# yezhen17/3DIoUMatch

Hardware: AMD Instinct MI355X
Metric: scenes/sec train-step (ScanNet 40k pts, 256 proposals) (higher is better)
Workload: dtype f32

## Files before the change

3dioumatch_amd/_lib.py:

```python
import ctypes
import os

_HERE = os.path.dirname(os.path.abspath(__file__))
LIB_PATH = os.path.join(_HERE, "lib3dioumatch_hip%s.so" % os.environ.get("PN2_LIB_SUFFIX", ""))

_c_int, _c_float, _vp, _sz = ctypes.c_int, ctypes.c_float, ctypes.c_void_p, ctypes.c_size_t


class MlpOperand(ctypes.Structure):
    _fields_ = [("mode", _c_int), ("x", _vp), ("dz", _vp), ("scale", _vp), ("shift", _vp), ("mean", _vp),
                ("invstd", _vp), ("coef", _vp), ("argmax", _vp), ("ns", _c_int), ("groups", _c_int),
                ("lin_w", _vp)]


_op = ctypes.POINTER(MlpOperand)

_SIGNATURES = {
    "pn2_furthest_point_sampling": [_c_int, _c_int, _c_int, _vp, _vp, _vp, _vp],
    "pn2_furthest_point_sampling_ws": [_c_int, _c_int, _c_int, _vp, _vp, _vp, _sz, _vp],
    "pn2_fps_workspace_bytes": [_c_int, _c_int, _c_int],
    "pn2_gather_points": [_c_int, _c_int, _c_int, _c_int, _vp, _vp, _vp, _vp],
    "pn2_gather_points_grad": [_c_int, _c_int, _c_int, _c_int, _vp, _vp, _vp, _vp],
    "pn2_ball_query": [_c_int, _c_int, _c_int, _c_float, _c_int, _vp, _vp, _vp, _vp, _sz, _vp],
    "pn2_ball_query_workspace_bytes": [_c_int, _c_int, _c_int, _c_int],
    "pn2_group_points": [_c_int, _c_int, _c_int, _c_int, _c_int, _vp, _vp, _vp, _vp],
    "pn2_group_points_grad": [_c_int, _c_int, _c_int, _c_int, _c_int, _vp, _vp, _vp, _vp],
    "pn2_three_nn": [_c_int, _c_int, _c_int, _vp, _vp, _vp, _vp, _vp],
    "pn2_three_interpolate": [_c_int, _c_int, _c_int, _c_int, _vp, _vp, _vp, _vp, _vp],
    "pn2_three_interpolate_affine_supported": [_c_int, _c_int, _c_int],
    "pn2_three_interpolate_affine": [_c_int, _c_int, _c_int, _c_int, _vp, _vp, _vp, _vp, _vp, _vp, _vp],
    "pn2_three_interpolate_affine_ld": [_c_int, _c_int, _c_int, _c_int, _vp, _vp, _vp, _vp, _c_int, _vp, _vp,
                                        _vp],
    "pn2_three_interpolate_rows_into": [_c_int, _c_int, _c_int, _c_int, _vp, _vp, _vp, _vp, _c_int, _c_int,
                                        _vp, _c_int, _c_int, _vp],
    "pn2_three_interpolate_grad": [_c_int, _c_int, _c_int, _c_int, _vp, _vp, _vp, _vp, _vp],
    "pn2_three_nn_weights": [ctypes.c_longlong, _vp, _vp, _vp],
    "pn2_multi_copy": [_c_int, _vp, ctypes.c_longlong, _vp],
    "pn2_group_inverse_supported": [_c_int, _c_int, _c_int],
    "pn2_group_inverse_entries": [_c_int, _c_int],
    "pn2_group_inverse_build": [_c_int, _c_int, _c_int, _c_int, _vp, _vp, _vp],
    "pn2_group_points_grad_sorted": [_c_int, _c_int, _c_int, _c_int, _c_int, _vp, _c_int, _c_int, _vp,
                                     _vp, _vp],
    "pn2_three_interpolate_into": [_c_int, _c_int, _c_int, _c_int, _vp, _vp, _vp, _vp, _c_int, _vp],
    "pn2_three_interpolate_grad_from": [_c_int, _c_int, _c_int, _c_int, _vp, _c_int, _vp, _vp, _vp, _vp],
    "pn2_query_and_group": [_c_int, _c_int, _c_int, _c_int, _c_float, _c_int, _c_int, _vp, _vp,
                            _vp, _vp, _vp, _vp, _sz, _vp],
    "pn2_group_concat": [_c_int, _c_int, _c_int, _c_int, _c_float, _c_int, _c_int, _vp, _vp,
                         _vp, _vp, _vp, _vp],
    "pn2_grid_bytes": [_c_int, _c_int],
    "pn2_grid_launch_order": [_c_int, _c_int, _vp, _vp, _vp, _vp],
    "pn2_grid_build": [_c_int, _c_int, _c_float, _vp, _vp, _sz, _vp],
    "pn2_ball_query_prebuilt": [_c_int, _c_int, _c_int, _c_float, _c_int, _vp, _vp, _vp, _vp, _sz, _vp],
    "pn2_query_and_group_prebuilt": [_c_int, _c_int, _c_int, _c_int, _c_float, _c_int, _c_int, _vp,
                                     _vp, _vp, _vp, _vp, _vp, _sz, _vp],
    "pn2_query_and_group_picks": [_c_int, _c_int, _c_int, _c_int, _c_float, _c_int, _c_int, _vp,
                                  _vp, _vp, _vp, _vp, _vp, _sz, _vp],
    "pn2_fps_grid_supported": [_c_int],
    "pn2_furthest_point_sampling_grid": [_c_int, _c_int, _c_int, _vp, _vp, _vp, _sz, _c_float, _vp,
                                         _sz, _vp],
    "pn2_fps_ties_supported": [_c_int],
    "pn2_furthest_point_sampling_ties": [_c_int, _c_int, _c_int, _vp, _vp, _vp, _sz, _c_float, _vp,
                                         _sz, _vp, _vp],
    "pn2_furthest_point_sampling_prefix": [_c_int, _c_int, _c_int, _vp, _vp, _vp, _sz, _vp, _vp],
    "pn2_error_string": [_c_int],
    "mlp_bn_workspace_floats": [_c_int, _c_int, _c_int],
    "mlp_bn_train_stats": [_c_int, _c_int, _c_int, _vp, _vp, _vp, _c_float, _c_float, _vp, _vp, _vp,
                           _vp, _vp, _vp, _vp, _vp, _vp],
    "mlp_bn_eval_coeff": [_c_int, _vp, _vp, _c_float, _vp, _vp, _vp, _vp, _vp, _vp, _vp],
    "mlp_bn_relu_apply": [_c_int, _c_int, _c_int, _vp, _vp, _vp, _vp, _vp],
    "mlp_bn_relu_pool": [_c_int, _c_int, _c_int, _c_int, _vp, _vp, _vp, _vp, _vp, _vp, _vp],
    "mlp_bn_relu_backward": [_c_int, _c_int, _c_int, _c_int, _vp, _vp, _vp, _vp, _vp, _vp, _vp, _vp,
                             _vp, _vp, _vp, _vp, _vp, _vp],
    "mlp_bn_relu_pool_backward": [_c_int, _c_int, _c_int, _c_int, _c_int, _vp, _vp, _vp, _vp, _vp,
                                  _vp, _vp, _vp, _vp, _vp, _vp, _vp, _vp, _vp, _vp, _vp],
    "mlp_bn_relu_backward_stats": [_c_int, _c_int, _c_int, _c_int, _vp, _vp, _vp, _vp, _vp, _vp,
                                   _vp, _vp, _vp, _vp, _vp, _vp, _vp],
    "mlp_gemm_forward": [_c_int] * 4 + [_vp, _vp, _op, _vp, _vp, _vp],
    "mlp_gemm_forward_small": [_c_int] * 4 + [_vp, _c_int, _vp, _op, _vp, _vp, _vp],
    "mlp_gemm_forward_stats_parts": [_c_int, _c_int, _c_int, _c_int, _vp],
    "mlp_bn_finalize_pairs": [_c_int, _c_int, _c_int, _vp, _vp, _vp, _c_float, _c_float, _vp, _vp,
                              _vp, _vp, _vp, _vp, _vp, _vp],
# ... 149 lines not shown
```

3dioumatch_amd/csrc/pn2_interp.hip:

```cpp
#include "common.h"

namespace {

constexpr int kNNTile = 1024;

__global__ void __launch_bounds__(256)
three_nn_kernel(int n, int m, const float *__restrict__ unknown,
                const float *__restrict__ known, float *__restrict__ dist2,
                int *__restrict__ idx) {
  __shared__ float4 tile[kNNTile];
  const BlockId blk = xcd_block_id();
  const int b = blk.y;
  const int j = blk.x * 256 + threadIdx.x;
  const bool live = j < n;
  const float *kn = known + (size_t)b * m * 3;
  float ux = 0.f, uy = 0.f, uz = 0.f;
  if (live) {
    const float *u = unknown + ((size_t)b * n + j) * 3;
    ux = u[0]; uy = u[1]; uz = u[2];
  }
  float best1 = __builtin_inff(), best2 = __builtin_inff(), best3 = __builtin_inff();
  int besti1 = 0, besti2 = 0, besti3 = 0;
  for (int base = 0; base < m; base += kNNTile) {
    const int cnt = m - base < kNNTile ? m - base : kNNTile;
// ... 145 lines not shown
                                 __fmul_rn(src[ii[t][1]], ww[t][1])),
                       __fmul_rn(src[ii[t][2]], ww[t][2]));
    float *dst = out + (size_t)b * out_bstride + (size_t)l * n + j0;
    if (JP == 4) {
      *reinterpret_cast<float4 *>(dst) = make_float4(r[0], r[1], r[2], r[3]);
    } else {
      dst[0] = r[0];
    }
  }
}

template <int CPW>
__global__ void __launch_bounds__(256)
three_interpolate_lds_kernel(int c, int m, int n, const float *__restrict__ points,
                             const int *__restrict__ idx, const float *__restrict__ weight,
                             float *__restrict__ out, size_t out_bstride, RowCopy rc) {
  extern __shared__ __attribute__((aligned(16))) float rows[];
  const BlockId blk = xcd_block_id();
  const int ygroups = (c + CPW - 1) / CPW;
  if (blk.y >= ygroups) {
    copy_rows<4>(rc, n, blk.z, blk.y - ygroups, (int)gridDim.y - ygroups, blk.x);
    return;
  }
  const int b = blk.z, l0 = blk.y * CPW;
  const int nc = c - l0 < CPW ? c - l0 : CPW;
  const float *src = points + ((size_t)b * c + l0) * m;
  for (int t = threadIdx.x; t < nc * m; t += 256) rows[t] = src[t];
  __syncthreads();
  const int j0 = (blk.x * 256 + threadIdx.x) * 4;
  if (j0 >= n) return;
  const int4 *ib = reinterpret_cast<const int4 *>(idx + ((size_t)b * n + j0) * 3);
  const float4 *wb = reinterpret_cast<const float4 *>(weight + ((size_t)b * n + j0) * 3);
  const int4 i0 = ib[0], i1 = ib[1], i2 = ib[2];
  const float4 w0 = wb[0], w1 = wb[1], w2 = wb[2];
  const int ii[12] = {i0.x, i0.y, i0.z, i0.w, i1.x, i1.y, i1.z, i1.w, i2.x, i2.y, i2.z, i2.w};
  const float ww[12] = {w0.x, w0.y, w0.z, w0.w, w1.x, w1.y, w1.z, w1.w, w2.x, w2.y, w2.z, w2.w};
#pragma unroll
  for (int cc = 0; cc < CPW; ++cc) {
    if (cc < nc) {
      const float *row = rows + cc * m;
      float r[4];
#pragma unroll
      for (int t = 0; t < 4; ++t)
        r[t] = __fadd_rn(__fadd_rn(__fmul_rn(row[ii[3 * t]], ww[3 * t]),
                                   __fmul_rn(row[ii[3 * t + 1]], ww[3 * t + 1])),
                         __fmul_rn(row[ii[3 * t + 2]], ww[3 * t + 2]));
      typedef float ti_f4 __attribute__((ext_vector_type(4)));
      __builtin_nontemporal_store(ti_f4{r[0], r[1], r[2], r[3]},
                                  reinterpret_cast<ti_f4 *>(out + (size_t)b * out_bstride + (size_t)(l0 + cc) * n + j0));
    }
  }
}

template <int CPW>
__global__ void __launch_bounds__(256)
three_interpolate_affine_lds_kernel(int c, int m, int n, const float *__restrict__ points,
                                    const int *__restrict__ idx, const float *__restrict__ weight,
                                    const float *__restrict__ aw, int aw_ld,
                                    const float *__restrict__ ax, float *__restrict__ out) {
  extern __shared__ __attribute__((aligned(16))) float rows[];
  const BlockId blk = xcd_block_id();
  const int b = blk.z, l0 = blk.y * CPW;
  const int nc = c - l0 < CPW ? c - l0 : CPW;
  const float *src = points + ((size_t)b * c + l0) * m;
  for (int t = threadIdx.x; t < nc * m; t += 256) rows[t] = src[t];
  __syncthreads();
  const int j0 = (blk.x * 256 + threadIdx.x) * 4;
  if (j0 >= n) return;
  const int4 *ib = reinterpret_cast<const int4 *>(idx + ((size_t)b * n + j0) * 3);
  const float4 *wb = reinterpret_cast<const float4 *>(weight + ((size_t)b * n + j0) * 3);
  const int4 i0 = ib[0], i1 = ib[1], i2 = ib[2];
  const float4 w0 = wb[0], w1 = wb[1], w2 = wb[2];
  const int ii[12] = {i0.x, i0.y, i0.z, i0.w, i1.x, i1.y, i1.z, i1.w, i2.x, i2.y, i2.z, i2.w};
  const float ww[12] = {w0.x, w0.y, w0.z, w0.w, w1.x, w1.y, w1.z, w1.w, w2.x, w2.y, w2.z, w2.w};
  const float *axb = ax + (size_t)b * 3 * n + j0;
  const float4 x0 = *reinterpret_cast<const float4 *>(axb), x1 = *reinterpret_cast<const float4 *>(axb + n),
               x2 = *reinterpret_cast<const float4 *>(axb + 2 * (size_t)n);
  const float xs[4][3] = {{x0.x, x1.x, x2.x}, {x0.y, x1.y, x2.y}, {x0.z, x1.z, x2.z}, {x0.w, x1.w, x2.w}};
#pragma unroll
  for (int cc = 0; cc < CPW; ++cc) {
    if (cc < nc) {
      const float *row = rows + cc * m;
      const float *awr = aw + (size_t)(l0 + cc) * aw_ld;
      const float a0 = awr[0], a1 = awr[1], a2 = awr[2];
      float r[4];
#pragma unroll
      for (int t = 0; t < 4; ++t) {
        const float interp = __fadd_rn(__fadd_rn(__fmul_rn(row[ii[3 * t]], ww[3 * t]),
                                                 __fmul_rn(row[ii[3 * t + 1]], ww[3 * t + 1])),
                                       __fmul_rn(row[ii[3 * t + 2]], ww[3 * t + 2]));
        const float affine = __fadd_rn(__fadd_rn(__fmul_rn(a0, xs[t][0]), __fmul_rn(a1, xs[t][1])),
                                       __fmul_rn(a2, xs[t][2]));
        r[t] = __fadd_rn(affine, interp);
      }
      typedef float ti_f4 __attribute__((ext_vector_type(4)));
      __builtin_nontemporal_store(ti_f4{r[0], r[1], r[2], r[3]},
                                  reinterpret_cast<ti_f4 *>(out + ((size_t)b * c + l0 + cc) * n + j0));
    }
  }
}

template <int CPW>
__global__ void __launch_bounds__(256)
three_interpolate_grad_lds_kernel(int c, int n, int m, const float *__restrict__ grad_out,
                                  size_t g_bstride, const int *__restrict__ idx,
                                  const float *__restrict__ weight,
                                  float *__restrict__ grad_points) {
  extern __shared__ __attribute__((aligned(16))) float lds[];
  const BlockId blk = xcd_block_id();
  const int b = blk.y, l0 = blk.x * CPW;
  const int nc = c - l0 < CPW ? c - l0 : CPW;
  for (int t = threadIdx.x; t < 4 * CPW * m; t += 256) lds[t] = 0.f;
  __syncthreads();
  float *rows = lds + (threadIdx.x >> 6) * CPW * m;
  for (int j = threadIdx.x; j < n; j += 256) {
    const int *ib = idx + ((size_t)b * n + j) * 3;
    const float *wb = weight + ((size_t)b * n + j) * 3;
    const int i1 = ib[0], i2 = ib[1], i3 = ib[2];
    const float w1 = wb[0], w2 = wb[1], w3 = wb[2];
#pragma unroll
    for (int cc = 0; cc < CPW; ++cc) {
      if (cc < nc) {
        const float g = grad_out[(size_t)b * g_bstride + (size_t)(l0 + cc) * n + j];
        float *row = rows + cc * m;
        atomicAdd(row + i1, __fmul_rn(g, w1));
        atomicAdd(row + i2, __fmul_rn(g, w2));
        atomicAdd(row + i3, __fmul_rn(g, w3));
      }
    }
  }
  __syncthreads();
  float *dst = grad_points + ((size_t)b * c + l0) * m;
  const int span = CPW * m;
  for (int t = threadIdx.x; t < nc * m; t += 256)
    dst[t] = __fadd_rn(__fadd_rn(__fadd_rn(lds[t], lds[span + t]), lds[2 * span + t]), lds[3 * span + t]);
}

__global__ void __launch_bounds__(256)
three_interpolate_grad_kernel(int c, int n, int m, const float *__restrict__ grad_out,
                              size_t g_bstride, const int *__restrict__ idx,
                              const float *__restrict__ weight, float *__restrict__ grad_points) {
  const BlockId blk = xcd_block_id();
  const int b = blk.z;
  const int j = blk.x * 256 + threadIdx.x;
  if (j >= n) return;
  const int *ib = idx + ((size_t)b * n + j) * 3;
  const float *wb = weight + ((size_t)b * n + j) * 3;
  const int i1 = ib[0], i2 = ib[1], i3 = ib[2];
  const float w1 = wb[0], w2 = wb[1], w3 = wb[2];
  for (int l = blk.y; l < c; l += gridDim.y) {
    const float g = grad_out[(size_t)b * g_bstride + (size_t)l * n + j];
// ... 41 lines not shown
    dim3 grid(pn2_ceil_div(n, 1024), pn2_ceil_div(c, CPW) + copy_groups, b);
    hipLaunchKernelGGL(three_interpolate_lds_kernel<CPW>, grid, dim3(256),
                       sizeof(float) * (size_t)CPW * m, stream, c, m, n, points, idx, weight, out,
                       out_bstride, rc);
    return pn2_launch_status();
  }
  const int ygroups = interp_channel_groups(c);
  if (vec) {
    dim3 grid(pn2_ceil_div(n, 1024), ygroups + copy_groups, b);
    hipLaunchKernelGGL(three_interpolate_kernel<4>, grid, dim3(256), 0, stream, c, m, n, points,
                       idx, weight, out, out_bstride, ygroups, rc);
  } else {
    dim3 grid(pn2_ceil_div(n, 256), ygroups + copy_groups, b);
    hipLaunchKernelGGL(three_interpolate_kernel<1>, grid, dim3(256), 0, stream, c, m, n, points,
                       idx, weight, out, out_bstride, ygroups, rc);
  }
  return pn2_launch_status();
}

static int interpolate_grad_run(int b, int c, int n, int m, const float *grad_out, size_t g_bstride,
                                const int *idx, const float *weight, float *grad_points,
                                hipStream_t stream) {
  if (b <= 0 || c <= 0 || m <= 0) return 0;
  if (n > 0 && m <= 1024) {
    constexpr int CPW = 4;
    hipLaunchKernelGGL(three_interpolate_grad_lds_kernel<CPW>, dim3(pn2_ceil_div(c, CPW), b),
                       dim3(256), sizeof(float) * 4 * (size_t)CPW * m, stream, c, n, m, grad_out,
                       g_bstride, idx, weight, grad_points);
    return pn2_launch_status();
  }
  const int e = pn2_zero_async(grad_points, sizeof(float) * (size_t)b * c * m, stream);
  if (e != 0) return e;
  if (n <= 0) return 0;
  dim3 grid(pn2_ceil_div(n, 256), interp_channel_groups(c), b);
  hipLaunchKernelGGL(three_interpolate_grad_kernel, grid, dim3(256), 0, stream, c, n, m, grad_out,
                     g_bstride, idx, weight, grad_points);
  return pn2_launch_status();
}

PN2_API int pn2_three_interpolate_affine_supported(int c, int m, int n) {
  return c > 0 && m > 0 && m <= 2048 && n >= 4 && n % 4 == 0;
}

PN2_API int pn2_three_interpolate_affine_ld(int b, int c, int m, int n, const float *points, const int *idx,
                                            const float *weight, const float *affine_w, int affine_w_ld,
                                            const float *affine_x, float *out, void *stream_) {
  if (b <= 0) return 0;
  if (!pn2_three_interpolate_affine_supported(c, m, n) || !affine_w || !affine_x || affine_w_ld < 3 ||
      (reinterpret_cast<size_t>(out) & 15) || (reinterpret_cast<size_t>(affine_x) & 15) ||
      (reinterpret_cast<size_t>(idx) & 15) || (reinterpret_cast<size_t>(weight) & 15))
    return (int)hipErrorInvalidValue;
  constexpr int CPW = 8;
  dim3 grid(pn2_ceil_div(n, 1024), pn2_ceil_div(c, CPW), b);
  hipLaunchKernelGGL(three_interpolate_affine_lds_kernel<CPW>, grid, dim3(256),
                     sizeof(float) * (size_t)CPW * m, (hipStream_t)stream_, c, m, n, points, idx, weight,
                     affine_w, affine_w_ld, affine_x, out);
  return pn2_launch_status();
}

PN2_API int pn2_three_interpolate_affine(int b, int c, int m, int n, const float *points, const int *idx,
                                         const float *weight, const float *affine_w,
                                         const float *affine_x, float *out, void *stream_) {
  return pn2_three_interpolate_affine_ld(b, c, m, n, points, idx, weight, affine_w, 3, affine_x, out,
                                         stream_);
}

PN2_API int pn2_three_interpolate(int b, int c, int m, int n, const float *points,
                                  const int *idx, const float *weight, float *out,
                                  void *stream_) {
  return interpolate_run(b, c, m, n, points, idx, weight, out, (size_t)c * n, (hipStream_t)stream_);
}

PN2_API int pn2_three_interpolate_grad(int b, int c, int n, int m, const float *grad_out,
                                       const int *idx, const float *weight, float *grad_points,
                                       void *stream_) {
  return interpolate_grad_run(b, c, n, m, grad_out, (size_t)c * n, idx, weight, grad_points,
                              (hipStream_t)stream_);
}

PN2_API int pn2_three_interpolate_into(int b, int c, int m, int n, const float *points,
                                       const int *idx, const float *weight, float *out,
                                       int c_total, void *stream_) {
  if (c_total < c) return (int)hipErrorInvalidValue;
  return interpolate_run(b, c, m, n, points, idx, weight, out, (size_t)c_total * n,
                         (hipStream_t)stream_);
}

PN2_API int pn2_three_interpolate_rows_into(int b, int c, int m, int n, const float *points,
                                            const int *idx, const float *weight, float *out,
                                            int c_total, int channel0, const float *rows, int rows_c,
                                            int rows_channel0, void *stream_) {
  if (b <= 0 || n <= 0) return 0;
  if (c <= 0 || rows_c <= 0 || !rows || channel0 < 0 || rows_channel0 < 0 ||
      channel0 + c > c_total || rows_channel0 + rows_c > c_total ||
      (channel0 < rows_channel0 + rows_c && rows_channel0 < channel0 + c))
    return (int)hipErrorInvalidValue;
  const size_t bstride = (size_t)c_total * n;
  const RowCopy rc = {rows, out + (size_t)rows_channel0 * n, rows_c, bstride};
  return interpolate_run(b, c, m, n, points, idx, weight, out + (size_t)channel0 * n, bstride,
                         (hipStream_t)stream_, rc);
}

PN2_API int pn2_three_interpolate_grad_from(int b, int c, int n, int m, const float *grad_out,
                                            int c_total, const int *idx, const float *weight,
                                            float *grad_points, void *stream_) {
  if (c_total < c) return (int)hipErrorInvalidValue;
  return interpolate_grad_run(b, c, n, m, grad_out, (size_t)c_total * n, idx, weight, grad_points,
                              (hipStream_t)stream_);
}
// ... 1 lines not shown
```

3dioumatch_amd/dropin/pointnet2/_ext.py:

```python
import importlib.util
import os
import sys

import torch


def _load_lib():
    name = "_3dioumatch_amd_lib"
    if name in sys.modules:
        return sys.modules[name]
    path = os.path.normpath(os.path.join(os.path.dirname(os.path.abspath(__file__)),
                                         "..", "..", "_lib.py"))
    spec = importlib.util.spec_from_file_location(name, path)
    mod = importlib.util.module_from_spec(spec)
    sys.modules[name] = mod
    try:
        spec.loader.exec_module(mod)
    except BaseException:
        del sys.modules[name]
        raise
    return mod


_L = _load_lib()
# ... 240 lines not shown
        raise RuntimeError("channel0 outside grad_out")
    if tuple(inverse.shape) != (b, _lib.pn2_group_inverse_entries(m, ns)) or not inverse.is_contiguous():
        raise RuntimeError("inverse is not the group_inverse() of a (B,%d,%d) index array" % (m, ns))
    out = torch.empty((b, c, int(n)), dtype=torch.float32, device=grad_out.device)
    with torch.cuda.device(grad_out.device):
        _L.check(_lib.pn2_group_points_grad_sorted(b, c, int(n), m, ns, grad_out.data_ptr(), c_total,
                                                   int(channel0), inverse.data_ptr(), out.data_ptr(),
                                                   _stream(grad_out)), "group_points_grad_sorted")
    return out


def three_interpolate_into(points, idx, weight, out, channel0):
    _chk_f32(points, "points"); _chk_i32(idx, "idx"); _chk_f32(weight, "weight"); _chk_f32(out, "out")
    _chk_dev(points, (idx, "idx"), (weight, "weight"), (out, "out"))
    b, c, m = points.shape
    n = idx.shape[1]
    c_total = out.shape[1]
    if out.shape[0] != b or out.shape[2] != n or channel0 < 0 or channel0 + c > c_total:
        raise RuntimeError("out must be (B, C_total >= channel0 + C, n)")
    with torch.cuda.device(points.device):
        _L.check(_lib.pn2_three_interpolate_into(b, c, m, n, points.data_ptr(), idx.data_ptr(),
                                                 weight.data_ptr(),
                                                 out.data_ptr() + 4 * channel0 * n, c_total,
                                                 _stream(points)), "three_interpolate_into")
    return out


def three_interpolate_rows_into(points, idx, weight, out, channel0, rows, rows_channel0):
    _chk_f32(points, "points"); _chk_i32(idx, "idx"); _chk_f32(weight, "weight"); _chk_f32(out, "out")
    _chk_f32(rows, "rows")
    _chk_dev(points, (idx, "idx"), (weight, "weight"), (out, "out"), (rows, "rows"))
    b, c, m = points.shape
    n = idx.shape[1]
    c_total, c_rows = out.shape[1], rows.shape[1]
    if out.shape[0] != b or out.shape[2] != n or channel0 < 0 or channel0 + c > c_total:
        raise RuntimeError("out must be (B, C_total >= channel0 + C, n)")
    if rows.dim() != 3 or rows.shape[0] != b or rows.shape[2] != n or rows_channel0 < 0 or \
            rows_channel0 + c_rows > c_total or \
            (channel0 < rows_channel0 + c_rows and rows_channel0 < channel0 + c):
        raise RuntimeError("rows must be (B, C_rows, n) and fit out's channels beside the interpolated block")
    with torch.cuda.device(points.device):
        _L.check(_lib.pn2_three_interpolate_rows_into(b, c, m, n, points.data_ptr(), idx.data_ptr(),
                                                      weight.data_ptr(), out.data_ptr(), c_total,
                                                      int(channel0), rows.data_ptr(), c_rows,
                                                      int(rows_channel0), _stream(points)),
                 "three_interpolate_rows_into")
    return out


def three_interpolate_affine_supported(c, m, n):
    return bool(_lib.pn2_three_interpolate_affine_supported(int(c), int(m), int(n)))


def three_interpolate_affine(points, idx, weight, affine_w, affine_x):
    for t, name in ((points, "points"), (weight, "weight"), (affine_x, "affine_x")):
        _chk_f32(t, name)
    if affine_w.dtype != torch.float32 or affine_w.dim() != 2 or affine_w.stride(1) != 1 or \
            affine_w.stride(0) < 3:
        raise RuntimeError("affine_w must be a float (C,3) matrix with contiguous rows")
    _chk_i32(idx, "idx")
    _chk_dev(points, (idx, "idx"), (weight, "weight"), (affine_w, "affine_w"), (affine_x, "affine_x"))
    b, c, m = points.shape
    n = idx.shape[1]
    if tuple(affine_w.shape) != (c, 3) or tuple(affine_x.shape) != (b, 3, n) or \
            not three_interpolate_affine_supported(c, m, n):
        raise RuntimeError("three_interpolate_affine: affine_w (C,3), affine_x (B,3,n), m <= 2048, n % 4 == 0")
    out = torch.empty((b, c, n), dtype=torch.float32, device=points.device)
    with torch.cuda.device(points.device):
        _L.check(_lib.pn2_three_interpolate_affine_ld(b, c, m, n, points.data_ptr(), idx.data_ptr(),
                                                      weight.data_ptr(), affine_w.data_ptr(),
                                                      int(affine_w.stride(0)), affine_x.data_ptr(),
                                                      out.data_ptr(), _stream(points)),
                 "three_interpolate_affine")
    return out


def three_interpolate_grad_from(grad, channel0, c, idx, weight, m):
    _chk_f32(grad, "grad"); _chk_i32(idx, "idx"); _chk_f32(weight, "weight")
    _chk_dev(grad, (idx, "idx"), (weight, "weight"))
    b, c_total, n = grad.shape
    out = torch.empty((b, int(c), int(m)), dtype=torch.float32, device=grad.device)
    with torch.cuda.device(grad.device):
        _L.check(_lib.pn2_three_interpolate_grad_from(b, int(c), n, int(m),
                                                      grad.data_ptr() + 4 * channel0 * n, c_total,
                                                      idx.data_ptr(), weight.data_ptr(),
                                                      out.data_ptr(), _stream(grad)),
                 "three_interpolate_grad_from")
    return out


def _ball_ws(t, b, n, m, nsample):
    need = int(_lib.pn2_ball_query_workspace_bytes(b, n, m, nsample))
    if need <= 0:
        return None, None, 0
    buf = torch.empty(need, dtype=torch.uint8, device=t.device)
    return buf, buf.data_ptr(), need


def ball_query(new_xyz, xyz, radius, nsample):
    _chk_f32(new_xyz, "new_xyz"); _chk_f32(xyz, "xyz"); _chk_dev(new_xyz, (xyz, "xyz"))
    b, n, _ = xyz.shape
    m = new_xyz.shape[1]
    nsample = int(nsample)
    if nsample <= 256 and b > 0 and m > 0:
        lists = _lists_for(xyz, radius)
        if lists is not None:
            return ball_query_prebuilt(new_xyz, xyz, radius, nsample, lists)
    idx = torch.empty((b, m, nsample), dtype=torch.int32, device=new_xyz.device)
    with torch.cuda.device(new_xyz.device):
        ws_buf, ws, ws_size = _ball_ws(new_xyz, b, n, m, nsample)
        _L.check(_lib.pn2_ball_query(b, n, m, float(radius), nsample, new_xyz.data_ptr(),
                                     xyz.data_ptr(), idx.data_ptr(), ws, ws_size,
                                     _stream(new_xyz)), "ball_query")
    return idx


def group_points(points, idx):
    _chk_f32(points, "points"); _chk_i32(idx, "idx"); _chk_dev(points, (idx, "idx"))
    b, c, n = points.shape
    _, m, ns = idx.shape
# ... 201 lines not shown
```

3dioumatch_amd/dropin/pointnet2/_mlp_ext.py:

```python
import contextlib
import ctypes
import os

import torch

from pointnet2._ext import _L, _lib, _stream

SMALL_BWD_DY_COLS = 4096


def _f32c(t, name):
    if t.dtype != torch.float32 or not t.is_contiguous() or not t.is_cuda:
        raise RuntimeError("%s must be a contiguous float32 GPU tensor" % name)


def _ws(y, b, c, r):
    n = int(_lib.mlp_bn_workspace_floats(b, c, r))
    return torch.empty(max(n, 1), dtype=torch.float32, device=y.device)


def new_tickets(channels, device):
    return torch.zeros(max(int(channels), 1), dtype=torch.int32, device=device)


# ... 225 lines not shown
            return e[2], e[3]
    return None


def gemm_forward(w, x, coeff=None, bias=None):
    _f32c(x, "x")
    b, k = x.shape[0], x.shape[1]
    r = x.numel() // (b * k)
    m = w.shape[0]
    sliced = w.dim() == 2 and not w.is_contiguous() and w.stride(1) == 1 and w.stride(0) >= k
    if sliced or bias is not None:
        if bias is not None:
            _f32c(bias, "bias")
        if _lib.mlp_gemm_image_supported(int(b), int(r)):
            if not sliced:
                _f32c(w, "w")
            elif w.dtype != torch.float32 or not w.is_cuda:
                raise RuntimeError("w must be a float32 GPU tensor")
            y = torch.empty((b, m) + tuple(x.shape[2:]), dtype=torch.float32, device=x.device)
            image = None if sliced else _image_of(w, b, r)
            op = _input_operand(x, coeff)
            with torch.cuda.device(x.device):
                _L.check(_lib.mlp_gemm_forward_small(b, m, k, r, w.data_ptr(),
                                                     int(w.stride(0)) if sliced else k,
                                                     image[0] if image else None, ctypes.byref(op),
                                                     _ptr(bias), y.data_ptr(), _stream(x)),
                         "mlp_gemm_forward_small")
            return y
        y = gemm_forward(w.contiguous(), x, coeff)
        if bias is not None:
            y += bias.view((1, -1) + (1,) * (y.dim() - 2))
        return y
    _f32c(w, "w")
    y = torch.empty((b, m) + tuple(x.shape[2:]), dtype=torch.float32, device=x.device)
    image = _image_of(w, b, r)
    op = _input_operand(x, coeff)
    with torch.cuda.device(x.device):
        _L.check(_lib.mlp_gemm_forward(b, m, k, r, w.data_ptr(), image[0] if image else None,
                                       ctypes.byref(op), y.data_ptr(), None, _stream(x)),
                 "mlp_gemm_forward")
    return y


def _finalize_pairs(c, parts, n_part, pairs, gamma, beta, running_mean, running_var, momentum, eps):
    out = torch.empty((4, c), dtype=torch.float32, device=pairs.device)
    scratch = torch.empty(int(_lib.mlp_bn_finalize_pairs_scratch_bytes(c)), dtype=torch.uint8,
                          device=pairs.device)
    _L.check(_lib.mlp_bn_finalize_pairs(c, parts, n_part, pairs.data_ptr(), gamma.data_ptr(),
                                        beta.data_ptr(), float(eps), float(momentum),
                                        _ptr(running_mean), _ptr(running_var), out[0].data_ptr(),
                                        out[1].data_ptr(), out[2].data_ptr(), out[3].data_ptr(),
                                        scratch.data_ptr(), _stream(pairs)), "mlp_bn_finalize_pairs")
    return out[0], out[1], out[2], out[3]


def gemm_forward_bn(w, x, coeff, gamma, beta, running_mean, running_var, momentum, eps, pool=False,
                    tickets=None, store=True):
    _f32c(x, "x"); _f32c(w, "w")
    b, k = x.shape[0], x.shape[1]
    r = x.numel() // (b * k)
    m = w.shape[0]
    cols = ctypes.c_int(0)
    parts = int(_lib.mlp_gemm_forward_stats_parts(b, m, k, r, ctypes.byref(cols)))
    if parts <= 0:
        y = gemm_forward(w, x, coeff)
        return (y,) + tuple(bn_coefficients(y, gamma, beta, running_mean, running_var, momentum,
                                            eps, True, tickets)) + ((None,) if pool else ())
    ns = x.shape[3] if (pool and x.dim() == 4) else 0
    pooled = bool(ns) and coeff is not None and w.data_ptr() % 16 == 0 and \
        bool(_lib.mlp_gemm_forward_stats_pool_supported(b, m, k, r, ns))
    ext = torch.empty((2, b, m, r // ns), dtype=torch.float32, device=x.device) if pooled else None
    if not store and not pooled:
        raise RuntimeError("gemm_forward_bn(store=False): the pooled epilogue does not cover this layer")
    y = torch.empty((b, m) + tuple(x.shape[2:]), dtype=torch.float32, device=x.device) if store else None
    pairs = torch.empty((parts, m, 2), dtype=torch.float32, device=x.device)
    op = _input_operand(x, coeff)
    with torch.cuda.device(x.device):
        if pooled:
            _L.check(_lib.mlp_gemm_forward_stats_pool(b, m, k, r, w.data_ptr(), ctypes.byref(op), _ptr(y),
                                                      pairs.data_ptr(), ns, gamma.data_ptr(),
                                                      ext.data_ptr(), _stream(x)),
                     "mlp_gemm_forward_stats_pool")
        else:
            _L.check(_lib.mlp_gemm_forward(b, m, k, r, w.data_ptr(), None, ctypes.byref(op),
                                           y.data_ptr(), pairs.data_ptr(), _stream(x)),
                     "mlp_gemm_forward(pairs)")
        bn = _finalize_pairs(m, parts, cols.value, pairs, gamma, beta, running_mean, running_var,
                             momentum, eps)
    return (y,) + bn + ((ext,) if pool else ())


def forward_pool_supported(w, x, coeff):
    shape = x if isinstance(x, tuple) else tuple(x.shape)
    if len(shape) != 4 or coeff is None or w.data_ptr() % 16 != 0:
        return False
    b, k, m, ns = shape
    return bool(_lib.mlp_gemm_forward_stats_pool_supported(b, w.shape[0], k, m * ns, ns))


def pool_from_extrema(ext, scale, shift):
    _, b, c, m = ext.shape
    pooled = torch.empty((b, c, m), dtype=torch.float32, device=ext.device)
    ymax = torch.empty_like(pooled)
    argmax = torch.empty((b, c, m), dtype=torch.int32, device=ext.device)
    with torch.cuda.device(ext.device):
        _L.check(_lib.mlp_bn_pool_from_extrema(b, c, m, ext.data_ptr(), scale.data_ptr(),
# ... 484 lines not shown
```

3dioumatch_amd/dropin/pointnet2/pytorch_utils.py:

```python
import contextlib
import os

import torch
import torch.nn as nn
from torch.autograd import Function


class _BNBase(nn.Sequential):

    def __init__(self, in_size, batch_norm=None, name=""):
        super().__init__()
        layer = batch_norm(in_size)
        nn.init.constant_(layer.weight, 1.0)
        nn.init.constant_(layer.bias, 0)
        self.add_module(name + "bn", layer)


class BatchNorm1d(_BNBase):
    def __init__(self, in_size, *, name=""):
        super().__init__(in_size, batch_norm=nn.BatchNorm1d, name=name)


class BatchNorm2d(_BNBase):
    def __init__(self, in_size, name=""):
# ... 70 lines not shown
        dy, dgamma, dbeta = K.bn_relu_backward(y, dz.contiguous(), gamma, scale, shift, mean,
                                               invstd, ctx.training, ctx.tickets)
        return dy, dgamma, dbeta, None, None, None, None, None, None


class _BNReLUMaxPool(Function):

    @staticmethod
    def forward(ctx, y, gamma, beta, running_mean, running_var, momentum, eps, training, tickets=None):
        from pointnet2 import _mlp_ext as K
        y = y.contiguous()
        mean, invstd, scale, shift = K.bn_coefficients(y, gamma, beta, running_mean, running_var,
                                                       momentum, eps, training, tickets)
        pooled, argmax, ymax = K.bn_relu_pool(y, scale, shift)
        ctx.save_for_backward(y, gamma, scale, shift, mean, invstd, argmax, ymax)
        ctx.training, ctx.tickets = training, tickets
        return pooled

    @staticmethod
    def backward(ctx, dpooled):
        from pointnet2 import _mlp_ext as K
        y, gamma, scale, shift, mean, invstd, argmax, ymax = ctx.saved_tensors
        dy, dgamma, dbeta = K.bn_relu_pool_backward(y, dpooled.contiguous(), argmax, ymax, gamma,
                                                    scale, shift, mean, invstd, ctx.training, ctx.tickets)
        return dy, dgamma, dbeta, None, None, None, None, None, None


class Pregathered(object):

    def __init__(self, idx, inverse, n):
        self.idx, self.inverse, self.n = idx, inverse, n
        self.extent = tuple(idx.shape)

    def forward(self, w, x, bn=None):
        from pointnet2 import _mlp_ext as K
        z = K.gemm_forward(w, x)
        return K.pregather_forward(z, self.idx, self.n, bn)

    def backward(self, w, x, fly, need_dx):
        from pointnet2 import _ext
        from pointnet2 import _mlp_ext as K
        inverse = self.inverse
        if inverse is None:
            inverse = _ext.group_inverse(self.idx, self.n)
        return K.both(w, x, need_dx=need_dx, dy=K.pregather_backward(fly, inverse, self.n))


class Interpolated(object):

    def __init__(self, idx, weight, rel, shape):
        self.idx, self.weight, self.rel, self.shape = idx, weight, rel, shape
        self.extent = (shape[0], shape[2], shape[3])

    def forward(self, w, x):
        from pointnet2 import _ext
        from pointnet2 import _mlp_ext as K
        z = K.gemm_forward(w[:, 3:], x)
        y = _ext.three_interpolate_affine(z, self.idx, self.weight, w[:, :3], self.rel)
        return y.view(self.shape)

    def input(self, x):
        from pointnet2 import _ext
        b, c = x.shape[0], 3 + x.shape[1]
        feats = torch.empty((b, c, self.rel.shape[2]), dtype=torch.float32, device=x.device)
        _ext.three_interpolate_rows_into(x, self.idx, self.weight, feats, 3, self.rel, 0)
        return feats.view(b, c, self.shape[2], self.shape[3])


def chain_forms(ws, x, pre, pool, training, input_grad):
    from pointnet2 import _mlp_ext as K
    n = len(ws)
    if pre is not None and (n < 2 or x.dim() != 3):
        raise RuntimeError("the pre-gather form needs src_ext (B, 3+C, n+m) and two layers or more")
    first = "plain"
    if isinstance(pre, Pregathered):
        first = "pregathered"
    elif isinstance(pre, Interpolated):
        first = "interpolated"
    elif training and n >= 3 and x.dim() == 4 and not input_grad and K.lin4_supported(ws[0], ws[1], x):
        chained = pool and n == 3 and K.chain_lin4_supported(ws[0], ws[1], ws[2], x, x.shape[3])
        first = "chained" if chained else "virtual"
    if not pool:
        return first, "apply"
    b, m, ns = pre.extent if pre is not None else (x.shape[0], x.shape[2], x.shape[3])
    y_in = (b, ws[-1].shape[1], m, ns)
    if first == "chained":
        return first, "gram" if K.pool_gram_supported(ws[2], y_in, ns) else "extrema"
    if not (training and n >= 2 and K.forward_pool_supported(ws[-1], y_in, True)):
        return first, "bn_relu_pool"
    return first, "gram" if K.pool_gram_supported(ws[-1], y_in, ns) else "extrema"


class _FusedMLPChain(Function):

    @staticmethod
    def forward(ctx, x, pool, training, momenta, epss, pre, tickets, *params):
        from pointnet2 import _mlp_ext as K
        n = len(params) // 5
        x = x.contiguous()
        ws = [w.reshape(w.shape[0], -1) for w in params[0::5]]
        bns = [tuple(params[5 * i + 1:5 * i + 5]) + (momenta[i], epss[i]) for i in range(n)]
        first, last = chain_forms(ws, x, pre, pool, training, ctx.needs_input_grad[0])
        store = any(ctx.needs_input_grad)
        ys, coefs = [], []
        moments, ext = None, None
        if first in ("virtual", "chained"):
            moments = K.first4_moments(x)
            ys.append(None)
            coefs.append(K.first4_bn(moments, x.numel() // 4, ws[0], *bns[0]))
        if first == "chained":
            y1, c1, y2, c2, ext = K.chain_lin4_forward(x, ws[0], coefs[0][2:], (ws[1],) + bns[1],
                                                       (ws[2],) + bns[2], store=store, store_last=last != "gram")
            ys += [y1, y2]
            coefs += [c1, c2]
        elif first == "virtual":
            y, *c = K.gemm_forward_bn_lin4(ws[1], x, ws[0], coefs[0][2:], *bns[1])
            ys.append(y)
            coefs.append(tuple(c))
        elif first == "pregathered" and training:
            y, *c = pre.forward(ws[0], x, bns[0])
            ys.append(y)
            coefs.append(tuple(c))
        elif pre is not None:
            ys.append(pre.forward(ws[0], x))
            coefs.append(K.bn_coefficients(ys[0], *bns[0], training, tickets))
        for i in range(len(ys), n):
            cur, coeff = (x, None) if i == 0 else (ys[i - 1], coefs[i - 1][2:])
            if i == n - 1 and last in ("extrema", "gram"):
                y, *c, ext = K.gemm_forward_bn(ws[i], cur, coeff, *bns[i], pool=True, tickets=tickets,
                                               store=store and last == "extrema")
            elif training:
                y, *c = K.gemm_forward_bn(ws[i], cur, coeff, *bns[i], tickets=tickets)
            else:
                y = K.gemm_forward(ws[i], cur, coeff)
                c = K.bn_coefficients(y, *bns[i], False, tickets)
            ys.append(y)
            coefs.append(tuple(c))
        scale, shift = coefs[-1][2:]
        argmax = ymax = None
        if last == "apply":
            out = K.bn_relu_apply(ys[-1], scale, shift)
        elif last == "bn_relu_pool":
            out, argmax, ymax = K.bn_relu_pool(ys[-1], scale, shift)
        else:
            out, argmax, ymax = K.pool_from_extrema(ext, scale, shift)
        ctx.save_for_backward(x, moments, argmax, ymax, *ys, *[t for c in coefs for t in c], *params)
        ctx.n_layers, ctx.training, ctx.tickets, ctx.pre = n, training, tickets, pre
        ctx.first, ctx.last = first, last
        return out

    @staticmethod
    def backward(ctx, dout):
        from pointnet2 import _mlp_ext as K
        n, training, tickets, first, last = ctx.n_layers, ctx.training, ctx.tickets, ctx.first, ctx.last
        x, moments, argmax, ymax, *rest = ctx.saved_tensors
        ys, rest = rest[:n], rest[n:]
        coefs, params = [tuple(rest[4 * i:4 * i + 4]) for i in range(n)], rest[4 * n:]
        ws = [w.reshape(w.shape[0], -1) for w in params[0::5]]
        if first == "interpolated":
            x = ctx.pre.input(x)
        need_dx, virtual = ctx.needs_input_grad[0], first in ("virtual", "chained")
        grads = [None] * (5 * n)
        dz, below = dout.contiguous(), None
        for i in range(n - 1, -1, -1):
            gamma = params[5 * i + 1]
            mean, invstd, scale, shift = coefs[i]
            if i == n - 1 and last == "gram":
                ns = ys[i - 1].shape[3]
                dgamma, dbeta, coef = K.bn_relu_pool_backward_stats(None, dz, argmax, ymax, gamma, scale, shift,
                                                                    mean, invstd, training, ns=ns,
                                                                    tickets=tickets)
                dz, dw, below = K.pool_gram_backward(ws[i], ys[i - 1], coefs[i - 1], params[5 * i - 4], coef,
# ... 347 lines not shown
```

include/pn2_hip.h:

```cpp
#ifndef PN2_HIP_H
#define PN2_HIP_H

#include <stddef.h>

#ifdef __cplusplus
extern "C" {
#endif

int pn2_furthest_point_sampling(int b, int n, int m, const float *dataset, float *temp,
                                int *idxs, void *stream);

int pn2_furthest_point_sampling_ws(int b, int n, int m, const float *dataset, int *idxs,
                                   void *workspace, size_t workspace_bytes, void *stream);
size_t pn2_fps_workspace_bytes(int b, int n, int m);

int pn2_gather_points(int b, int c, int n, int npoints, const float *points, const int *idx,
                      float *out, void *stream);

int pn2_gather_points_grad(int b, int c, int n, int npoints, const float *grad_out,
                           const int *idx, float *grad_points, void *stream);

int pn2_ball_query(int b, int n, int m, float radius, int nsample, const float *new_xyz,
                   const float *xyz, int *idx, void *workspace, size_t workspace_bytes,
                   void *stream);
size_t pn2_ball_query_workspace_bytes(int b, int n, int m, int nsample);

int pn2_group_points(int b, int c, int n, int npoints, int nsample, const float *points,
                     const int *idx, float *out, void *stream);

int pn2_group_points_grad(int b, int c, int n, int npoints, int nsample, const float *grad_out,
                          const int *idx, float *grad_points, void *stream);

int pn2_three_nn(int b, int n, int m, const float *unknown, const float *known, float *dist2,
                 int *idx, void *stream);

int pn2_three_interpolate(int b, int c, int m, int n, const float *points, const int *idx,
                          const float *weight, float *out, void *stream);

int pn2_three_interpolate_affine_supported(int c, int m, int n);
int pn2_three_interpolate_affine(int b, int c, int m, int n, const float *points, const int *idx,
                                 const float *weight, const float *affine_w, const float *affine_x,
                                 float *out, void *stream);
int pn2_three_interpolate_affine_ld(int b, int c, int m, int n, const float *points, const int *idx,
                                    const float *weight, const float *affine_w, int affine_w_ld,
                                    const float *affine_x, float *out, void *stream);

int pn2_three_interpolate_grad(int b, int c, int n, int m, const float *grad_out,
                               const int *idx, const float *weight, float *grad_points,
                               void *stream);

int pn2_three_interpolate_into(int b, int c, int m, int n, const float *points, const int *idx,
                               const float *weight, float *out, int c_total, void *stream);
int pn2_three_interpolate_rows_into(int b, int c, int m, int n, const float *points, const int *idx,
                                    const float *weight, float *out, int c_total, int channel0,
                                    const float *rows, int rows_c, int rows_channel0, void *stream);
int pn2_three_interpolate_grad_from(int b, int c, int n, int m, const float *grad_out, int c_total,
                                    const int *idx, const float *weight, float *grad_points,
                                    void *stream);


int pn2_query_and_group(int b, int n, int m, int c, float radius, int nsample, int normalize_xyz,
                        const float *new_xyz, const float *xyz, const float *features,
                        int *idx, float *out, void *workspace, size_t workspace_bytes,
                        void *stream);

int pn2_group_concat(int b, int n, int m, int c, float radius, int nsample, int normalize_xyz,
                     const float *new_xyz, const float *xyz, const float *features,
                     const int *idx, float *out, void *stream);


size_t pn2_grid_bytes(int b, int n);

int pn2_grid_launch_order(int b, int n, size_t *start_offset, int *start_stride,
                          int *order_for_slot, size_t *order_offset);

int pn2_grid_build(int b, int n, float radius, const float *xyz, void *grid, size_t grid_bytes,
                   void *stream);

int pn2_ball_query_prebuilt(int b, int n, int m, float radius, int nsample, const float *new_xyz,
                            const float *xyz, int *idx, const void *grid, size_t grid_bytes,
                            void *stream);

int pn2_query_and_group_prebuilt(int b, int n, int m, int c, float radius, int nsample,
                                 int normalize_xyz, const float *new_xyz, const float *xyz,
                                 const float *features, int *idx, float *out, const void *grid,
                                 size_t grid_bytes, void *stream);

int pn2_query_and_group_picks(int b, int n, int m, int c, float radius, int nsample,
                              int normalize_xyz, const float *new_xyz, const float *xyz,
                              const float *features, int *idx, float *out, const void *grid,
                              size_t grid_bytes, void *stream);

int pn2_fps_grid_supported(int n);

int pn2_furthest_point_sampling_grid(int b, int n, int m, const float *dataset, int *idxs,
                                     void *workspace, size_t workspace_bytes, float grid_radius,
                                     void *grid, size_t grid_bytes, void *stream);

// ... 27 lines not shown
```

Before: 1426.

## Fuse batchnorm partial statistics into affine three-interpolate kernel for FP layers

Adds a STATS variant of the affine three-interpolate LDS kernel that, after writing each output tile, computes per-channel shifted mean/variance partials over its 1024 points with wave reductions. These pairs are passed to an existing BN finalize routine, so the first MLP layer after feature propagation no longer needs a separate pass over the interpolated output to compute batch statistics. It applies only when n is a multiple of 1024. The cost is extra syncs, LDS use and registers to hold the outputs in the kernel.

```diff
diff --git a/3dioumatch_amd/_lib.py b/3dioumatch_amd/_lib.py
--- a/3dioumatch_amd/_lib.py
+++ b/3dioumatch_amd/_lib.py
@@ -27,6 +27,9 @@
     "pn2_group_points_grad": [_c_int, _c_int, _c_int, _c_int, _c_int, _vp, _vp, _vp, _vp],
     "pn2_three_nn": [_c_int, _c_int, _c_int, _vp, _vp, _vp, _vp, _vp],
     "pn2_three_interpolate": [_c_int, _c_int, _c_int, _c_int, _vp, _vp, _vp, _vp, _vp],
+    "pn2_three_interpolate_affine_pairs_supported": [_c_int, _c_int, _c_int],
+    "pn2_three_interpolate_affine_pairs": [_c_int, _c_int, _c_int, _c_int, _vp, _vp, _vp, _vp, _c_int, _vp, _vp,
+                                           _vp, _vp],
     "pn2_three_interpolate_affine_supported": [_c_int, _c_int, _c_int],
     "pn2_three_interpolate_affine": [_c_int, _c_int, _c_int, _c_int, _vp, _vp, _vp, _vp, _vp, _vp, _vp],
     "pn2_three_interpolate_affine_ld": [_c_int, _c_int, _c_int, _c_int, _vp, _vp, _vp, _vp, _c_int, _vp, _vp,
diff --git a/3dioumatch_amd/csrc/pn2_interp.hip b/3dioumatch_amd/csrc/pn2_interp.hip
--- a/3dioumatch_amd/csrc/pn2_interp.hip
+++ b/3dioumatch_amd/csrc/pn2_interp.hip
@@ -221,12 +221,13 @@
   }
 }
 
-template <int CPW>
+template <int CPW, bool STATS>
 __global__ void __launch_bounds__(256)
 three_interpolate_affine_lds_kernel(int c, int m, int n, const float *__restrict__ points,
                                     const int *__restrict__ idx, const float *__restrict__ weight,
                                     const float *__restrict__ aw, int aw_ld,
-                                    const float *__restrict__ ax, float *__restrict__ out) {
+                                    const float *__restrict__ ax, float *__restrict__ out,
+                                    float *__restrict__ pairs) {
   extern __shared__ __attribute__((aligned(16))) float rows[];
   const BlockId blk = xcd_block_id();
   const int b = blk.z, l0 = blk.y * CPW;
@@ -246,13 +247,14 @@
   const float4 x0 = *reinterpret_cast<const float4 *>(axb), x1 = *reinterpret_cast<const float4 *>(axb + n),
                x2 = *reinterpret_cast<const float4 *>(axb + 2 * (size_t)n);
   const float xs[4][3] = {{x0.x, x1.x, x2.x}, {x0.y, x1.y, x2.y}, {x0.z, x1.z, x2.z}, {x0.w, x1.w, x2.w}};
+  float keep[STATS ? CPW : 1][4] = {};
 #pragma unroll
   for (int cc = 0; cc < CPW; ++cc) {
     if (cc < nc) {
       const float *row = rows + cc * m;
       const float *awr = aw + (size_t)(l0 + cc) * aw_ld;
       const float a0 = awr[0], a1 = awr[1], a2 = awr[2];
-      float r[4];
+      float *r = keep[STATS ? cc : 0];
 #pragma unroll
       for (int t = 0; t < 4; ++t) {
         const float interp = __fadd_rn(__fadd_rn(__fmul_rn(row[ii[3 * t]], ww[3 * t]),
@@ -266,6 +268,33 @@
       __builtin_nontemporal_store(ti_f4{r[0], r[1], r[2], r[3]},
                                   reinterpret_cast<ti_f4 *>(out + ((size_t)b * c + l0 + cc) * n + j0));
     }
+  }
+  if (!STATS) return;
+  __syncthreads();
+  float *first = rows, *wsum = rows + CPW;
+  if (threadIdx.x == 0) {
+#pragma unroll
+    for (int cc = 0; cc < CPW; ++cc) first[cc] = keep[cc][0];
+  }
+  __syncthreads();
+  const int lane = lane_id(), w = threadIdx.x / kWave;
+#pragma unroll
+  for (int cc = 0; cc < CPW; ++cc) {
+    const float sh = first[cc];
+    const float d0 = keep[cc][0] - sh, d1 = keep[cc][1] - sh, d2 = keep[cc][2] - sh, d3 = keep[cc][3] - sh;
+    const float s1 = wave_sum((d0 + d1) + (d2 + d3));
+    const float s2 = wave_sum((d0 * d0 + d1 * d1) + (d2 * d2 + d3 * d3));
+    if (lane == 0) { wsum[(w * 2 + 0) * CPW + cc] = s1; wsum[(w * 2 + 1) * CPW + cc] = s2; }
+  }
+  __syncthreads();
+  if ((int)threadIdx.x < nc) {
+    const int cc = threadIdx.x;
+    const float s1 = ((wsum[cc] + wsum[2 * CPW + cc]) + wsum[4 * CPW + cc]) + wsum[6 * CPW + cc];
+    const float s2 = ((wsum[CPW + cc] + wsum[3 * CPW + cc]) + wsum[5 * CPW + cc]) + wsum[7 * CPW + cc];
+    const float fn = 1024.f;
+    float *o = pairs + (((size_t)b * gridDim.x + blk.x) * c + l0 + cc) * 2;
+    o[0] = first[cc] + s1 / fn;
+    o[1] = fmaxf(s2 - s1 * s1 / fn, 0.f);
   }
 }
 
@@ -413,9 +442,32 @@
     return (int)hipErrorInvalidValue;
   constexpr int CPW = 8;
   dim3 grid(pn2_ceil_div(n, 1024), pn2_ceil_div(c, CPW), b);
-  hipLaunchKernelGGL(three_interpolate_affine_lds_kernel<CPW>, grid, dim3(256),
+  hipLaunchKernelGGL((three_interpolate_affine_lds_kernel<CPW, false>), grid, dim3(256),
                      sizeof(float) * (size_t)CPW * m, (hipStream_t)stream_, c, m, n, points, idx, weight,
-                     affine_w, affine_w_ld, affine_x, out);
+                     affine_w, affine_w_ld, affine_x, out, nullptr);
+  return pn2_launch_status();
+}
+
+PN2_API int pn2_three_interpolate_affine_pairs_supported(int c, int m, int n) {
+  return pn2_three_interpolate_affine_supported(c, m, n) && n % 1024 == 0;
+}
+
+PN2_API int pn2_three_interpolate_affine_pairs(int b, int c, int m, int n, const float *points,
+                                               const int *idx, const float *weight, const float *affine_w,
+                                               int affine_w_ld, const float *affine_x, float *out,
+                                               float *pairs, void *stream_) {
+  if (b <= 0) return 0;
+  if (!pn2_three_interpolate_affine_pairs_supported(c, m, n) || !affine_w || !affine_x || affine_w_ld < 3 ||
+      !pairs || (reinterpret_cast<size_t>(pairs) & 7) ||
+      (reinterpret_cast<size_t>(out) & 15) || (reinterpret_cast<size_t>(affine_x) & 15) ||
+      (reinterpret_cast<size_t>(idx) & 15) || (reinterpret_cast<size_t>(weight) & 15))
+    return (int)hipErrorInvalidValue;
+  constexpr int CPW = 8;
+  dim3 grid(n / 1024, pn2_ceil_div(c, CPW), b);
+  const size_t lds_floats = (size_t)CPW * (m > 9 ? m : 9);
+  hipLaunchKernelGGL((three_interpolate_affine_lds_kernel<CPW, true>), grid, dim3(256),
+                     sizeof(float) * lds_floats, (hipStream_t)stream_, c, m, n, points, idx, weight,
+                     affine_w, affine_w_ld, affine_x, out, pairs);
   return pn2_launch_status();
 }
 
diff --git a/3dioumatch_amd/dropin/pointnet2/_ext.py b/3dioumatch_amd/dropin/pointnet2/_ext.py
--- a/3dioumatch_amd/dropin/pointnet2/_ext.py
+++ b/3dioumatch_amd/dropin/pointnet2/_ext.py
@@ -316,7 +316,11 @@
     return bool(_lib.pn2_three_interpolate_affine_supported(int(c), int(m), int(n)))
 
 
-def three_interpolate_affine(points, idx, weight, affine_w, affine_x):
+def three_interpolate_affine_pairs_supported(c, m, n):
+    return bool(_lib.pn2_three_interpolate_affine_pairs_supported(int(c), int(m), int(n)))
+
+
+def three_interpolate_affine(points, idx, weight, affine_w, affine_x, pairs=False):
     for t, name in ((points, "points"), (weight, "weight"), (affine_x, "affine_x")):
         _chk_f32(t, name)
     if affine_w.dtype != torch.float32 or affine_w.dim() != 2 or affine_w.stride(1) != 1 or \
@@ -330,6 +334,18 @@
             not three_interpolate_affine_supported(c, m, n):
         raise RuntimeError("three_interpolate_affine: affine_w (C,3), affine_x (B,3,n), m <= 2048, n % 4 == 0")
     out = torch.empty((b, c, n), dtype=torch.float32, device=points.device)
+    if pairs:
+        if not three_interpolate_affine_pairs_supported(c, m, n):
+            raise RuntimeError("three_interpolate_affine(pairs=True): n must be a multiple of 1024")
+        parts = torch.empty((b * (n // 1024), c, 2), dtype=torch.float32, device=points.device)
+        with torch.cuda.device(points.device):
+            _L.check(_lib.pn2_three_interpolate_affine_pairs(b, c, m, n, points.data_ptr(), idx.data_ptr(),
+                                                             weight.data_ptr(), affine_w.data_ptr(),
+                                                             int(affine_w.stride(0)), affine_x.data_ptr(),
+                                                             out.data_ptr(), parts.data_ptr(),
+                                                             _stream(points)),
+                     "three_interpolate_affine_pairs")
+        return out, parts
     with torch.cuda.device(points.device):
         _L.check(_lib.pn2_three_interpolate_affine_ld(b, c, m, n, points.data_ptr(), idx.data_ptr(),
                                                       weight.data_ptr(), affine_w.data_ptr(),
diff --git a/3dioumatch_amd/dropin/pointnet2/_mlp_ext.py b/3dioumatch_amd/dropin/pointnet2/_mlp_ext.py
--- a/3dioumatch_amd/dropin/pointnet2/_mlp_ext.py
+++ b/3dioumatch_amd/dropin/pointnet2/_mlp_ext.py
@@ -301,6 +301,13 @@
                                         out[1].data_ptr(), out[2].data_ptr(), out[3].data_ptr(),
                                         scratch.data_ptr(), _stream(pairs)), "mlp_bn_finalize_pairs")
     return out[0], out[1], out[2], out[3]
+
+
+def finalize_pairs(pairs, n_part, gamma, beta, running_mean, running_var, momentum, eps):
+    _f32c(pairs, "pairs")
+    with torch.cuda.device(pairs.device):
+        return _finalize_pairs(pairs.shape[1], pairs.shape[0], int(n_part), pairs, gamma, beta,
+                               running_mean, running_var, momentum, eps)
 
 
 def gemm_forward_bn(w, x, coeff, gamma, beta, running_mean, running_var, momentum, eps, pool=False,
diff --git a/3dioumatch_amd/dropin/pointnet2/pytorch_utils.py b/3dioumatch_amd/dropin/pointnet2/pytorch_utils.py
--- a/3dioumatch_amd/dropin/pointnet2/pytorch_utils.py
+++ b/3dioumatch_amd/dropin/pointnet2/pytorch_utils.py
@@ -146,12 +146,20 @@
         self.idx, self.weight, self.rel, self.shape = idx, weight, rel, shape
         self.extent = (shape[0], shape[2], shape[3])
 
-    def forward(self, w, x):
+    def leaves_pairs(self, w, x):
         from pointnet2 import _ext
+        pairs_ok = getattr(_ext, "three_interpolate_affine_pairs_supported", None)
+        return pairs_ok is not None and pairs_ok(w.shape[0], x.shape[2], self.idx.shape[1])
+
+    def forward(self, w, x, bn=None):
+        from pointnet2 import _ext
         from pointnet2 import _mlp_ext as K
         z = K.gemm_forward(w[:, 3:], x)
-        y = _ext.three_interpolate_affine(z, self.idx, self.weight, w[:, :3], self.rel)
-        return y.view(self.shape)
+        if bn is None:
+            y = _ext.three_interpolate_affine(z, self.idx, self.weight, w[:, :3], self.rel)
+            return y.view(self.shape)
+        y, pairs = _ext.three_interpolate_affine(z, self.idx, self.weight, w[:, :3], self.rel, pairs=True)
+        return (y.view(self.shape),) + K.finalize_pairs(pairs, 1024, *bn)
 
     def input(self, x):
         from pointnet2 import _ext
@@ -211,7 +219,7 @@
             y, *c = K.gemm_forward_bn_lin4(ws[1], x, ws[0], coefs[0][2:], *bns[1])
             ys.append(y)
             coefs.append(tuple(c))
-        elif first == "pregathered" and training:
+        elif pre is not None and training and (first == "pregathered" or pre.leaves_pairs(ws[0], x)):
             y, *c = pre.forward(ws[0], x, bns[0])
             ys.append(y)
             coefs.append(tuple(c))
diff --git a/include/pn2_hip.h b/include/pn2_hip.h
--- a/include/pn2_hip.h
+++ b/include/pn2_hip.h
@@ -44,6 +44,10 @@
 int pn2_three_interpolate_affine_ld(int b, int c, int m, int n, const float *points, const int *idx,
                                     const float *weight, const float *affine_w, int affine_w_ld,
                                     const float *affine_x, float *out, void *stream);
+int pn2_three_interpolate_affine_pairs_supported(int c, int m, int n);
+int pn2_three_interpolate_affine_pairs(int b, int c, int m, int n, const float *points, const int *idx,
+                                       const float *weight, const float *affine_w, int affine_w_ld,
+                                       const float *affine_x, float *out, float *pairs, void *stream);
 
 int pn2_three_interpolate_grad(int b, int c, int n, int m, const float *grad_out,
                                const int *idx, const float *weight, float *grad_points,
```

Result: no change. 1427, median of 2 (+0.1%).
